# Hi-PACE/hipace

Hardware: AMD Instinct MI355X
Metric: transverse slices/s at 1024^2 x 4ppc (explicit solver) (higher is better)
Workload: dtype f64

## Files before the change

hipace_amd/csrc/multigrid.hip:

```cpp
#include "common.h"
#include <type_traits>
#include "mg_gate.h"
#include "slab_ops.h"

#include <vector>
#include <algorithm>
#include <cmath>
#include <cstring>

namespace hps {

struct FView {
    double* p; long js, ns; int oi, oj;
    __device__ __forceinline__ double& operator() (int i, int j, int n) const {
        const unsigned o = (unsigned)((i + oi) + (j + oj)*(int)js + n*(int)ns)*8u;
        return *reinterpret_cast<double*>(reinterpret_cast<char*>(p) + o);
    }
};

struct LevBox { int lox, loy, hix, hiy;
                int vlx, vly, vhx, vhy; };

enum { SRC_ZERO = 0, SRC_DIRECT = 1, SRC_PROLONG = 2 };

#define HPS_KEEP(x) asm volatile("" :: "v"(x))

#ifdef HPS_STAMPS
__device__ long long* g_mg_dbg = nullptr;
#define MG_STAMP(i) do { if (g_mg_dbg && blockIdx.x == 0 && threadIdx.x == 0) g_mg_dbg[i] = __builtin_amdgcn_s_memtime(); } while (0)
#else
#define MG_STAMP(i) do { } while (0)
#endif

template <int TX_, int TY_, int NT_>
struct TileShape {
    static constexpr int TX = TX_, TY = TY_, NT = NT_;
    static constexpr int AX = TX + 2, AY = TY + 2;
    static constexpr int PR = TX/2;
    static constexpr int GPAIRS = TX*TY/2/NT;
    static_assert(TX*TY/2 % NT == 0 && NT % 64 == 0 && (PR == 16 || PR == 32), "tile shape");
};
using TileBig = TileShape<64, 32, 512>;
using TileMid = TileShape<32, 32, 256>;
using TileHuge = TileShape<64, 48, 512>;
using TileHugeNodal = TileShape<64, 32, 512>;
template <bool CC> struct HugeTileOf { using type = TileHuge; };
template <> struct HugeTileOf<false> { using type = TileHugeNodal; };
using TileSmall = TileShape<32, 16, 256>;

template <bool CC>
__device__ __forceinline__ double diag_c0 (int i, int j, const LevBox& b, double acf, double facx, double facy)
{
    double c0 = -(acf + 2.0*(facx + facy));
    if (CC && (i == b.lox || i == b.hix)) c0 -= 2.0*facx;
    if (CC && (j == b.loy || j == b.hiy)) c0 -= 2.0*facy;
    return c0;
}

template <bool CC, bool INTERIOR = false, class P>
__device__ __forceinline__ double offdiag (P c, int sy, int i, int j, const LevBox& b, double facx, double facy)
{
    const double w = c[-1], e = c[1], s = c[-sy], n = c[sy];
    double lx = facx*(w + e), ly = facy*(s + n);
    if (CC && !INTERIOR) {
        const double fx43 = facx*(4./3.), fy43 = facy*(4./3.);
        lx = (i == b.lox) ? fx43*e : ((i == b.hix) ? fx43*w : lx);
        ly = (j == b.loy) ? fy43*n : ((j == b.hiy) ? fy43*s : ly);
    }
    return lx + ly;
}
// ... 32 lines not shown
    }
    lap += tx;
    lap += ty;
    return rhs + acf*p0 - lap;
}

template <bool CC>
__device__ __forceinline__ double prolong_at (const FView& crse, int i, int j, int n)
{
    const int ic = i >> 1, jc = j >> 1;
    if (CC) return crse(ic, jc, n);
    const bool io = (i & 1), jo = (j & 1);
    if (io && jo)  return (crse(ic, jc, n) + crse(ic+1, jc, n) + crse(ic, jc+1, n) + crse(ic+1, jc+1, n))*0.25;
    if (io)        return (crse(ic, jc, n) + crse(ic+1, jc, n))*0.5;
    if (jo)        return (crse(ic, jc, n) + crse(ic, jc+1, n))*0.5;
    return crse(ic, jc, n);
}

constexpr int MG_MAX_VCYCLES = 1024;
template <int NT>
__device__ __forceinline__ void block_max_to (unsigned long long* slot, double v, double* s_red)
{
    for (int o = 32; o > 0; o >>= 1) v = fmax(v, __shfl_xor(v, o));
    if ((threadIdx.x & 63) == 0) s_red[threadIdx.x >> 6] = v;
    __syncthreads();
    if (threadIdx.x == 0) {
        double m = 0.0;
        for (int w = 0; w < NT/64; ++w) m = fmax(m, s_red[w]);
        if (m > 0.0) atomicMax(slot + (blockIdx.x & (MG_NSUB - 1)), (unsigned long long)__double_as_longlong(m));
    }
    __syncthreads();
}

#define MG_ROWPK(m) const int jj = BR ? (tid / PR)*GPAIRS + (m) : (tid + MG_NT*(m)) / PR, pk = BR ? (tid & (PR - 1)) : (tid + MG_NT*(m)) - jj*PR
template <bool CC> __device__ __forceinline__ double restrict_at (const FView& fine, int i, int j, int n);
template <class TS, bool CC, int SRC, bool DO_RES, bool FUSE_R, bool INTERIOR, int NSW, bool GATE_IN = (NSW == 4), bool RPULL = false>
__device__ __forceinline__ void smooth_tile (double (&s_phi)[2][TS::AY*TS::AX], double* s_red, double* s_crs, const LevBox& b, const FView& phi_out,
                                             const FView& phi_out2, const FView& rhs, const FView& acf, const FView& phi_in, const FView& crse,
                                             const FView& res_out, const FView& cres_out, double facx, double facy,
                                             int gi0, int gj0, unsigned long long* resnorm, unsigned long long* rhsnorm, const StopRule& sr)
{
    constexpr int E = DO_RES ? NSW : NSW - 1;
    constexpr int GT_X = TS::TX, GT_Y = TS::TY, GA_X = TS::AX, GA_Y = TS::AY, MG_NT = TS::NT, GPAIRS = TS::GPAIRS, PR = TS::PR;
    constexpr int AXH = GA_X/2, CH = GA_Y*AXH;
    constexpr bool BR = GPAIRS <= 2 || INTERIOR;
    const int tid = threadIdx.x;
    const int cpar = (gi0 + gj0) & 1;
    MG_STAMP(0);
    double r0[GPAIRS][2], r1[GPAIRS][2], ac[GPAIRS][2], ci[GPAIRS][2];
    bool in[GPAIRS][2];
    int hx[GPAIRS];
    double fxm[GPAIRS][2], fym[GPAIRS];
    double rmax = 0.0;
#pragma unroll
    for (int m = 0; m < GPAIRS; ++m) {
        MG_ROWPK(m);
        const int j = gj0 + jj;
        hx[m] = (gi0 + 2*pk + j) & 1;
        fym[m] = INTERIOR ? facy : wall_mult<CC>(j, b.loy, b.hiy, facy);
#pragma unroll
        for (int p = 0; p < 2; ++p) {
            const int i = gi0 + 2*pk + (hx[m] ^ p);
            fxm[m][p] = INTERIOR ? facx : wall_mult<CC>(i, b.lox, b.hix, facx);
            const int ic = INTERIOR ? i : min(max(i, b.vlx), b.vhx), jc = INTERIOR ? j : min(max(j, b.vly), b.vhy);
            const bool ok = INTERIOR || (ic == i && jc == j);
            in[m][p] = ok;
            double a0, a1;
            if constexpr (RPULL) { a0 = restrict_at<CC>(crse, ic, jc, 0); a1 = restrict_at<CC>(crse, ic, jc, 1); }
            else { a0 = rhs(ic, jc, 0); a1 = rhs(ic, jc, 1); }
            const double a2 = acf(ic, jc, 0);
            r0[m][p] = ok ? a0 : 0.0;
            r1[m][p] = ok ? a1 : 0.0;
            ac[m][p] = ok ? a2 : 0.0;
            ci[m][p] = 1.0/diag_c0<CC>(i, j, b, ac[m][p], facx, facy);
            if (rhsnorm) rmax = fmax(rmax, fmax(fabs(r0[m][p]), fabs(r1[m][p])));
        }
    }
    MG_STAMP(1);
    {
        constexpr int NF = (GA_X*GA_Y + MG_NT - 1)/MG_NT;
        double v0[NF], v1[NF];
        constexpr bool PLDS = !CC && SRC == SRC_PROLONG;
        constexpr int CXN = GA_X/2 + 2, CYN = GA_Y/2 + 2;
        const int cx0 = (INTERIOR ? gi0 - 1 : min(max(gi0 - 1, b.vlx), b.vhx)) >> 1, cy0 = (INTERIOR ? gj0 - 1 : min(max(gj0 - 1, b.vly), b.vhy)) >> 1;
        if constexpr (PLDS) {
            const int cxl = b.vlx >> 1, cxh = (b.vhx >> 1) + 1, cyl = b.vly >> 1, cyh = (b.vhy >> 1) + 1;
            constexpr int NC = (CXN*CYN + MG_NT - 1)/MG_NT;
            double c0[NC], c1[NC];
#pragma unroll
            for (int m = 0; m < NC; ++m) {
                const int q = min(tid + MG_NT*m, CXN*CYN - 1);
                const int ly = q / CXN, lx = q - ly*CXN;
                const int X = min(max(cx0 + lx, cxl), cxh), Y = min(max(cy0 + ly, cyl), cyh);
                c0[m] = crse(X, Y, 0); c1[m] = crse(X, Y, 1);
            }
#pragma unroll
            for (int m = 0; m < NC; ++m) {
                const int q = tid + MG_NT*m;
                if (q < CXN*CYN) { s_crs[q] = c0[m]; s_crs[CXN*CYN + q] = c1[m]; }
            }
        }
#pragma unroll
        for (int m = 0; m < NF; ++m) {
            const int s = min(tid + MG_NT*m, GA_X*GA_Y - 1);
            const int lj = s / GA_X, li = s - lj*GA_X;
            const int i = gi0 - 1 + li, j = gj0 - 1 + lj;
            v0[m] = 0.0; v1[m] = 0.0;
            if (SRC != SRC_ZERO) {
                const int ic = INTERIOR ? i : min(max(i, b.vlx), b.vhx), jc = INTERIOR ? j : min(max(j, b.vly), b.vhy);
                double a0 = phi_in(ic, jc, 0), a1 = phi_in(ic, jc, 1);
                if (SRC == SRC_PROLONG && !PLDS) { a0 += prolong_at<CC>(crse, ic, jc, 0); a1 += prolong_at<CC>(crse, ic, jc, 1); }
                const bool inside = INTERIOR || (ic == i && jc == j);
                v0[m] = inside ? a0 : 0.0; v1[m] = inside ? a1 : 0.0;
            }
        }
        if constexpr (PLDS) {
            __syncthreads();
#pragma unroll
            for (int m = 0; m < NF; ++m) {
                const int s = min(tid + MG_NT*m, GA_X*GA_Y - 1);
                const int lj = s / GA_X, li = s - lj*GA_X;
                const int i = gi0 - 1 + li, j = gj0 - 1 + lj;
                const int ic = INTERIOR ? i : min(max(i, b.vlx), b.vhx), jc = INTERIOR ? j : min(max(j, b.vly), b.vhy);
                const bool inside = INTERIOR || (ic == i && jc == j);
                const int o = ((jc >> 1) - cy0)*CXN + (ic >> 1) - cx0;
                const bool io = (ic & 1), jo = (jc & 1);
                double p0, p1;
                const double* q0 = s_crs + o; const double* q1 = s_crs + CXN*CYN + o;
                if (io && jo)  { p0 = (q0[0] + q0[1] + q0[CXN] + q0[CXN + 1])*0.25; p1 = (q1[0] + q1[1] + q1[CXN] + q1[CXN + 1])*0.25; }
                else if (io)   { p0 = (q0[0] + q0[1])*0.5; p1 = (q1[0] + q1[1])*0.5; }
                else if (jo)   { p0 = (q0[0] + q0[CXN])*0.5; p1 = (q1[0] + q1[CXN])*0.5; }
                else           { p0 = q0[0]; p1 = q1[0]; }
                if (inside) { v0[m] += p0; v1[m] += p1; }
            }
        }
        {
            if (GATE_IN) {
                const bool active = vcycle_active(sr);
#pragma unroll
                for (int m = 0; m < GPAIRS; ++m) { HPS_KEEP(r0[m][0]); HPS_KEEP(r0[m][1]); HPS_KEEP(r1[m][0]); HPS_KEEP(r1[m][1]); HPS_KEEP(ac[m][0]); HPS_KEEP(ac[m][1]); }
#pragma unroll
                for (int m = 0; m < NF; ++m) { HPS_KEEP(v0[m]); HPS_KEEP(v1[m]); }
                if (!active) return;
            }
        }
#pragma unroll
        for (int m = 0; m < NF; ++m) {
            const int s = tid + MG_NT*m;
            if (s < GA_X*GA_Y) {
                const int lj = s / GA_X, li = s - lj*GA_X;
                const int o = ((cpar + li + lj) & 1)*CH + lj*AXH + (li >> 1);
                s_phi[0][o] = v0[m]; s_phi[1][o] = v1[m];
            }
        }
    }
    __syncthreads();
    MG_STAMP(2);

    double l0[GPAIRS][2], l1[GPAIRS][2];
    if constexpr (BR) {
#pragma unroll
        for (int m = 0; m < GPAIRS; ++m) {
            MG_ROWPK(m);
            const int row = (jj + 1)*AXH + pk;
#pragma unroll
            for (int p = 0; p < 2; ++p) { const int h = hx[m] ^ p; l0[m][p] = s_phi[0][p*CH + row + h]; l1[m][p] = s_phi[1][p*CH + row + h]; }
        }
#pragma unroll
        for (int icolor = 0; icolor < NSW; ++icolor) {
            const int p = icolor & 1;
#pragma unroll
            for (int m = 0; m < GPAIRS; ++m) {
                MG_ROWPK(m);
                const int h = hx[m] ^ p;
                const int row = (jj + 1)*AXH + pk;
                const double* nb0 = &s_phi[0][(1 - p)*CH + row];
                const double* nb1 = &s_phi[1][(1 - p)*CH + row];
                const double we0 = nb0[h] + l0[m][1 - p], we1 = nb1[h] + l1[m][1 - p];
                const double s0 = (m > 0) ? l0[m > 0 ? m - 1 : 0][1 - p] : nb0[h - AXH], s1 = (m > 0) ? l1[m > 0 ? m - 1 : 0][1 - p] : nb1[h - AXH];
                const double t0 = (m + 1 < GPAIRS) ? l0[m + 1 < GPAIRS ? m + 1 : m][1 - p] : nb0[h + AXH], t1 = (m + 1 < GPAIRS) ? l1[m + 1 < GPAIRS ? m + 1 : m][1 - p] : nb1[h + AXH];
                const double n0 = (r0[m][p] - (fxm[m][p]*we0 + fym[m]*(s0 + t0)))*ci[m][p];
                const double n1 = (r1[m][p] - (fxm[m][p]*we1 + fym[m]*(s1 + t1)))*ci[m][p];
                if (INTERIOR || in[m][p]) { s_phi[0][p*CH + row + h] = n0; s_phi[1][p*CH + row + h] = n1; l0[m][p] = n0; l1[m][p] = n1; }
            }
            __syncthreads();
        }
    } else {
#pragma unroll
        for (int icolor = 0; icolor < NSW; ++icolor) {
            constexpr int dummy = 0; (void)dummy;
            const int p = icolor & 1;
#pragma unroll
            for (int m = 0; m < GPAIRS; ++m) {
                MG_ROWPK(m);
                const int h = hx[m] ^ p;
                const int row = (jj + 1)*AXH + pk;
                const double* nb0 = &s_phi[0][(1 - p)*CH + row];
                const double* nb1 = &s_phi[1][(1 - p)*CH + row];
                const double n0 = (r0[m][p] - (fxm[m][p]*(nb0[0] + nb0[1]) + fym[m]*(nb0[h - AXH] + nb0[h + AXH])))*ci[m][p];
                const double n1 = (r1[m][p] - (fxm[m][p]*(nb1[0] + nb1[1]) + fym[m]*(nb1[h - AXH] + nb1[h + AXH])))*ci[m][p];
                if (INTERIOR || in[m][p]) { s_phi[0][p*CH + row + h] = n0; s_phi[1][p*CH + row + h] = n1; }
            }
            __syncthreads();
        }
    }
    MG_STAMP(3);

    double resmax = 0.0;
    if constexpr (BR) {
        double la0[GPAIRS], ra0[GPAIRS], la1[GPAIRS], ra1[GPAIRS];
        bool finr[GPAIRS];
#pragma unroll
        for (int m = 0; m < GPAIRS; ++m) {
            MG_ROWPK(m);
            const int j = gj0 + jj;
            const bool rowok = (jj >= E && jj < GT_Y - E);
            double q0[2], q1[2];
            bool fin[2];
#pragma unroll
            for (int p = 0; p < 2; ++p) {
                const int h = hx[m] ^ p;
                const int ii = 2*pk + h;
                fin[p] = rowok && ii >= E && ii < GT_X - E && in[m][p];
                const int i = gi0 + ii;
                const int row = (jj + 1)*AXH + pk;
                const double f0 = l0[m][p], f1 = l1[m][p];
                q0[p] = 0.0; q1[p] = 0.0;
                if (DO_RES) {
                    const double* nb0 = &s_phi[0][(1 - p)*CH + row];
                    const double* nb1 = &s_phi[1][(1 - p)*CH + row];
                    const double o0 = nb0[h], o1 = nb1[h];
                    const double w0 = h ? l0[m][1 - p] : o0, e0 = h ? o0 : l0[m][1 - p];
                    const double w1 = h ? l1[m][1 - p] : o1, e1 = h ? o1 : l1[m][1 - p];
                    const double s0 = (m > 0) ? l0[m > 0 ? m - 1 : 0][1 - p] : nb0[h - AXH], s1 = (m > 0) ? l1[m > 0 ? m - 1 : 0][1 - p] : nb1[h - AXH];
                    const double n0 = (m + 1 < GPAIRS) ? l0[m + 1 < GPAIRS ? m + 1 : m][1 - p] : nb0[h + AXH], n1 = (m + 1 < GPAIRS) ? l1[m + 1 < GPAIRS ? m + 1 : m][1 - p] : nb1[h + AXH];
                    const double t0 = residual_v<INTERIOR>(f0, w0, e0, s0, n0, i, j, b, r0[m][p], ac[m][p], facx, facy);
                    const double t1 = residual_v<INTERIOR>(f1, w1, e1, s1, n1, i, j, b, r1[m][p], ac[m][p], facx, facy);
                    q0[p] = fin[p] ? t0 : 0.0; q1[p] = fin[p] ? t1 : 0.0;
                    resmax = fmax(resmax, fmax(fabs(q0[p]), fabs(q1[p])));
                }
                if (fin[p]) {
                    if constexpr (RPULL) { rhs(i, j, 0) = r0[m][p]; rhs(i, j, 1) = r1[m][p]; }
                    if (DO_RES && !FUSE_R) { res_out(i, j, 0) = q0[p]; res_out(i, j, 1) = q1[p]; }
                    phi_out(i, j, 0) = f0;
                    phi_out(i, j, 1) = f1;
                    if (phi_out2.p) { phi_out2(i, j, 0) = f0; phi_out2(i, j, 1) = f1; }
                }
            }
            const bool sw = (hx[m] != 0);
            la0[m] = sw ? q0[1] : q0[0]; ra0[m] = sw ? q0[0] : q0[1];
            la1[m] = sw ? q1[1] : q1[0]; ra1[m] = sw ? q1[0] : q1[1];
            finr[m] = fin[0];
        }
        if (FUSE_R) {
            const double c0 = __shfl_down(la0[0], PR), d0 = __shfl_down(ra0[0], PR);
            const double c1 = __shfl_down(la1[0], PR), d1 = __shfl_down(ra1[0], PR);
#pragma unroll
            for (int m = 0; m < GPAIRS; ++m) {
                MG_ROWPK(m);
                if (finr[m] && ((jj & 1) == 0)) {
                    const bool own = (m + 1 < GPAIRS);
                    const int mu = own ? m + 1 : m;
                    const double ua0 = own ? la0[mu] : c0, ub0 = own ? ra0[mu] : d0, ua1 = own ? la1[mu] : c1, ub1 = own ? ra1[mu] : d1;
                    const int ic = (gi0 + 2*pk) >> 1, jc = (gj0 + jj) >> 1;
                    cres_out(ic, jc, 0) = 0.25*(la0[m] + ra0[m] + ua0 + ub0);
                    cres_out(ic, jc, 1) = 0.25*(la1[m] + ra1[m] + ua1 + ub1);
                }
            }
        }
    } else {
#pragma unroll
        for (int m = 0; m < GPAIRS; ++m) {
            MG_ROWPK(m);
            const int j = gj0 + jj;
            const bool rowok = (jj >= E && jj < GT_Y - E);
            double q0[2], q1[2];
            bool fin[2];
#pragma unroll
            for (int p = 0; p < 2; ++p) {
                const int h = hx[m] ^ p;
                const int ii = 2*pk + h;
                fin[p] = rowok && ii >= E && ii < GT_X - E && in[m][p];
                const int i = gi0 + ii;
                const int row = (jj + 1)*AXH + pk;
                const double f0 = s_phi[0][p*CH + row + h], f1 = s_phi[1][p*CH + row + h];
                q0[p] = 0.0; q1[p] = 0.0;
                if (DO_RES) {
                    const double* nb0 = &s_phi[0][(1 - p)*CH + row];
                    const double* nb1 = &s_phi[1][(1 - p)*CH + row];
                    const double t0 = residual_v<INTERIOR>(f0, nb0[0], nb0[1], nb0[h - AXH], nb0[h + AXH], i, j, b, r0[m][p], ac[m][p], facx, facy);
                    const double t1 = residual_v<INTERIOR>(f1, nb1[0], nb1[1], nb1[h - AXH], nb1[h + AXH], i, j, b, r1[m][p], ac[m][p], facx, facy);
                    q0[p] = fin[p] ? t0 : 0.0; q1[p] = fin[p] ? t1 : 0.0;
                    resmax = fmax(resmax, fmax(fabs(q0[p]), fabs(q1[p])));
                }
                if (fin[p]) {
                    if constexpr (RPULL) { rhs(i, j, 0) = r0[m][p]; rhs(i, j, 1) = r1[m][p]; }
                    if (DO_RES && !FUSE_R) { res_out(i, j, 0) = q0[p]; res_out(i, j, 1) = q1[p]; }
                    phi_out(i, j, 0) = f0;
                    phi_out(i, j, 1) = f1;
                    if (phi_out2.p) { phi_out2(i, j, 0) = f0; phi_out2(i, j, 1) = f1; }
                }
            }
            if (FUSE_R) {
                const bool sw = (hx[m] != 0);
                const double la0 = sw ? q0[1] : q0[0], ra0 = sw ? q0[0] : q0[1];
                const double la1 = sw ? q1[1] : q1[0], ra1 = sw ? q1[0] : q1[1];
                const double c0 = __shfl_down(la0, PR), d0 = __shfl_down(ra0, PR);
                const double c1 = __shfl_down(la1, PR), d1 = __shfl_down(ra1, PR);
                if (fin[0] && ((tid & PR) == 0)) {
                    const int ic = (gi0 + 2*pk) >> 1, jc = j >> 1;
                    cres_out(ic, jc, 0) = 0.25*(la0 + ra0 + c0 + d0);
                    cres_out(ic, jc, 1) = 0.25*(la1 + ra1 + c1 + d1);
                }
            }
        }
    }
    MG_STAMP(4);
    if (DO_RES && resnorm) block_max_to<MG_NT>(resnorm, resmax, s_red);
    if (rhsnorm) block_max_to<MG_NT>(rhsnorm, rmax, s_red);
    MG_STAMP(5);
}

template <class TS, bool CC, int SRC, bool DO_RES, bool FUSE_R, int NSW = 4, bool RPULL = false>
__global__ __launch_bounds__(TS::NT, (RPULL && TS::GPAIRS > 1) ? 2 : 4)
void k_smooth (LevBox b, FView phi_out, FView phi_out2, FView rhs, FView acf, FView phi_in, FView crse, FView res_out,
               FView cres_out, double facx, double facy, int ntx, unsigned long long* resnorm,
               unsigned long long* rhsnorm, StopRule sr)
{
    static_assert(!FUSE_R || (CC && DO_RES), "fused restriction is cell-centred only");
    if (NSW != 4 && !vcycle_active(sr)) return;
    constexpr int GT_X = TS::TX, GT_Y = TS::TY;
    __shared__ double s_phi[2][TS::AY*TS::AX];
    __shared__ double s_red[TS::NT/64];
    constexpr bool PLDS = !CC && SRC == SRC_PROLONG;
    __shared__ double s_crs[PLDS ? 2*(TS::AX/2 + 2)*(TS::AY/2 + 2) : 1];
    constexpr int E = DO_RES ? NSW : NSW - 1;
    constexpr int FX = GT_X - 2*E, FY = GT_Y - 2*E;
    const int nb = gridDim.x, q8 = nb >> 3, r8 = nb & 7, xcd = blockIdx.x & 7;
    const int tile = xcd*q8 + min(xcd, r8) + (blockIdx.x >> 3);
    const int bx = tile % ntx, by = tile / ntx;
    const int gi0 = b.vlx + bx*FX - E;
    const int gj0 = b.vly + by*FY - E;
    const bool interior = (gi0 - 1 >= b.vlx) && (gi0 + GT_X <= b.vhx) && (gj0 - 1 >= b.vly) && (gj0 + GT_Y <= b.vhy)
                       && (gi0 > b.lox) && (gi0 + GT_X - 1 < b.hix) && (gj0 > b.loy) && (gj0 + GT_Y - 1 < b.hiy);
    constexpr bool GATE_IN = (NSW == 4);
    if (interior) smooth_tile<TS, CC, SRC, DO_RES, FUSE_R, true, NSW, GATE_IN, RPULL>(s_phi, s_red, s_crs, b, phi_out, phi_out2, rhs, acf, phi_in, crse, res_out, cres_out,
                                                             facx, facy, gi0, gj0, resnorm, rhsnorm, sr);
    else          smooth_tile<TS, CC, SRC, DO_RES, FUSE_R, false, NSW, GATE_IN, RPULL>(s_phi, s_red, s_crs, b, phi_out, phi_out2, rhs, acf, phi_in, crse, res_out, cres_out,
                                                              facx, facy, gi0, gj0, resnorm, rhsnorm, sr);
}

template <bool CC>
__device__ __forceinline__ double restrict_at (const FView& fine, int i, int j, int n)
{
    if (CC) return 0.25*(fine(2*i, 2*j, n) + fine(2*i+1, 2*j, n) + fine(2*i, 2*j+1, n) + fine(2*i+1, 2*j+1, n));
    return (1./16.)*(fine(2*i-1, 2*j-1, n) + 2.*fine(2*i, 2*j-1, n) + fine(2*i+1, 2*j-1, n)
                   + 2.*fine(2*i-1, 2*j, n) + 4.*fine(2*i, 2*j, n) + 2.*fine(2*i+1, 2*j, n)
                   + fine(2*i-1, 2*j+1, n) + 2.*fine(2*i, 2*j+1, n) + fine(2*i+1, 2*j+1, n));
}

template <bool CC>
__global__ __launch_bounds__(256)
void k_restrict (LevBox cb, FView crse, FView fine, int ncomp, StopRule sr)
{
    if (!vcycle_active(sr)) return;
    const int i = cb.vlx + blockIdx.x*blockDim.x + threadIdx.x;
    const int j = cb.vly + blockIdx.y;
    if (i > cb.vhx || j > cb.vhy) return;
    for (int n = 0; n < ncomp; ++n) crse(i, j, n) = restrict_at<CC>(fine, i, j, n);
}

typedef __attribute__((address_space(3))) double lds_double;

struct LowLev { LevBox b; int nxb; int cells; int off; };

struct LView {
    lds_double* p; int nxb; int lox, loy;
    __device__ __forceinline__ lds_double& operator() (int i, int j) const { return p[(i - lox) + (j - loy)*nxb]; }
};
__device__ __forceinline__ LView lplane (lds_double* base, const LowLev& l, int plane)
{
    return LView{base + l.off + plane*l.cells, l.nxb, l.b.lox, l.b.loy};
}

template <bool CC>
__device__ __forceinline__ double lrestrict (const LView& f, int i, int j)
{
    if (CC) return 0.25*(f(2*i, 2*j) + f(2*i+1, 2*j) + f(2*i, 2*j+1) + f(2*i+1, 2*j+1));
    return (1./16.)*(f(2*i-1, 2*j-1) + 2.*f(2*i, 2*j-1) + f(2*i+1, 2*j-1)
                   + 2.*f(2*i-1, 2*j) + 4.*f(2*i, 2*j) + 2.*f(2*i+1, 2*j)
                   + f(2*i-1, 2*j+1) + 2.*f(2*i, 2*j+1) + f(2*i+1, 2*j+1));
}

template <bool CC>
__device__ __forceinline__ double lprolong (const LView& c, int i, int j)
{
    const int ic = i >> 1, jc = j >> 1;
    if (CC) return c(ic, jc);
    const bool io = (i & 1), jo = (j & 1);
    if (io && jo)  return (c(ic, jc) + c(ic+1, jc) + c(ic, jc+1) + c(ic+1, jc+1))*0.25;
    if (io)        return (c(ic, jc) + c(ic+1, jc))*0.5;
    if (jo)        return (c(ic, jc) + c(ic, jc+1))*0.5;
// ... 857 lines not shown
            e.total = off3;
            HPS_HIP_CHECK(hipMalloc(&M->coef_img, (size_t)e.ctot*sizeof(double)));
            HPS_HIP_CHECK(hipMemset(M->coef_img, 0, (size_t)e.ctot*sizeof(double)));
            M->low3_lds = (size_t)off3*sizeof(double);
            if (M->low3_lds > 64*1024)
                HPS_HIP_CHECK(hipFuncSetAttribute((const void*)k_lower_v3, hipFuncAttributeMaxDynamicSharedMemorySize, (int)M->low3_lds));
            HPS_HIP_CHECK(hipMalloc(&M->d_low3, sizeof(Low2)));
            HPS_HIP_CHECK(hipMemcpy(M->d_low3, &e, sizeof(Low2), hipMemcpyHostToDevice));
            HPS_HIP_CHECK(hipMalloc(&M->cinvA, (size_t)e.nx[0]*e.ny[0]*sizeof(double)));
            break;
        }
    }
    if (!M->use_low3) {
        long cells = 0;
        for (int il = M->lowv_begin; il < nl; ++il) cells += M->L[il].cells;
        M->low_lds = (size_t)(8*cells)*sizeof(double);
        hipFuncAttributes fa{};
        HPS_HIP_CHECK(hipFuncGetAttributes(&fa, M->cc ? (const void*)k_lower_v<true> : (const void*)k_lower_v<false>));
        if (M->low_lds + fa.sharedSizeBytes > device_max_lds()) { M->bottom = true; M->lowv_begin = nl - 1; M->low_lds = 0; }
    }
    M->nodal_pull1 = !M->cc && M->lowv_begin > 1;
    if (!M->use_low3 && !M->bottom) {
        std::vector<LowLev> low;
        int off = 0;
        for (int il = M->lowv_begin; il < nl; ++il) {
            const MGLevelDev& l = M->L[il];
            low.push_back(LowLev{l.b, l.b.hix - l.b.lox + 1, (int)l.cells, off});
            off += 8*(int)l.cells;
        }
        if (M->low_lds > 64*1024) {
            HPS_HIP_CHECK(hipFuncSetAttribute((const void*)k_lower_v<true>, hipFuncAttributeMaxDynamicSharedMemorySize, (int)M->low_lds));
            HPS_HIP_CHECK(hipFuncSetAttribute((const void*)k_lower_v<false>, hipFuncAttributeMaxDynamicSharedMemorySize, (int)M->low_lds));
        }
        HPS_HIP_CHECK(hipMalloc(&M->d_low, low.size()*sizeof(LowLev)));
        HPS_HIP_CHECK(hipMemcpy(M->d_low, low.data(), low.size()*sizeof(LowLev), hipMemcpyHostToDevice));
    }
    HPS_HIP_CHECK(hipMalloc(&M->d_buf, (3 + MG_MAX_VCYCLES)*MG_NSUB*sizeof(unsigned long long)));
    HPS_HIP_CHECK(hipHostMalloc(&M->h_buf, ((3 + MG_MAX_VCYCLES)*MG_NSUB + 8)*sizeof(unsigned long long), hipHostMallocMapped));
    HPS_HIP_CHECK(hipHostGetDevicePointer((void**)&M->h_buf_dev, M->h_buf, 0));
    M->h_seq = M->h_buf + (3 + MG_MAX_VCYCLES)*MG_NSUB; M->h_seq_dev = M->h_buf_dev + (3 + MG_MAX_VCYCLES)*MG_NSUB;
    *M->h_seq = 0ULL;
    HPS_HIP_CHECK(hipMemset(M->d_buf, 0, (3 + MG_MAX_VCYCLES)*MG_NSUB*sizeof(unsigned long long)));
    memset(M->h_buf, 0, (3 + MG_MAX_VCYCLES)*MG_NSUB*sizeof(unsigned long long));
    M->d_norms = M->d_buf + MG_NSUB; M->h_norms = M->h_buf + MG_NSUB;
    HPS_HIP_CHECK(hipMalloc(&M->tmp0, 2*M->L[0].cells*sizeof(double)));
    HPS_HIP_CHECK(hipMemset(M->tmp0, 0, 2*M->L[0].cells*sizeof(double)));
    *out = M;
    return HPS_OK;
}

template <class TS, bool CC, int SRC, bool DO_RES, int NSW = 4, bool RPULL = false>
static void launch_smooth_ts (Multigrid* M, int il, FView phi_out, FView phi_out2, FView rhs, FView acf, FView phi_in, FView crse,
                              FView res_out, FView cres_out, unsigned long long* resnorm, unsigned long long* rhsnorm,
                              const StopRule& sr, hipStream_t st)
{
    const LevBox& b = M->L[il].b;
    constexpr int E = DO_RES ? NSW : NSW - 1;
    constexpr int FX = TS::TX - 2*E, FY = TS::TY - 2*E;
    const int ntx = ceil_div(b.vhx - b.vlx + 1, FX), nty = ceil_div(b.vhy - b.vly + 1, FY);
    const double fac = (double)(1 << il);
    const double ldx = M->dx*fac, ldy = M->dy*fac;
    const double facx = 1.0/(ldx*ldx), facy = 1.0/(ldy*ldy);
    constexpr bool FUSE = CC && DO_RES;
    hipLaunchKernelGGL((k_smooth<TS, CC, SRC, DO_RES, FUSE, NSW, RPULL>), dim3(ntx*nty), dim3(TS::NT), 0, st, b, phi_out, phi_out2, rhs, acf,
                       phi_in, crse, res_out, cres_out, facx, facy, ntx, resnorm, rhsnorm, sr);
}

template <bool CC, int SRC, bool DO_RES>
static void launch_smooth (Multigrid* M, int il, FView phi_out, FView phi_out2, FView rhs, FView acf, FView phi_in, FView crse,
                           FView res_out, FView cres_out, unsigned long long* resnorm, unsigned long long* rhsnorm,
                           const StopRule& sr, hipStream_t st)
{
    if (M->L[il].cells <= SMALL_TILE_CELLS)
        launch_smooth_ts<TileSmall, CC, SRC, DO_RES>(M, il, phi_out, phi_out2, rhs, acf, phi_in, crse, res_out, cres_out, resnorm, rhsnorm, sr, st);
    else
        launch_smooth_ts<TileBig, CC, SRC, DO_RES>(M, il, phi_out, phi_out2, rhs, acf, phi_in, crse, res_out, cres_out, resnorm, rhsnorm, sr, st);
}

template <bool CC>
static void restrict_residual_if_nodal (Multigrid* M, int il, const StopRule& sr, hipStream_t st)
{
    if (CC) return;
    const LevBox& cb = M->L[il+1].b;
    hipLaunchKernelGGL(k_restrict<CC>, dim3(ceil_div(cb.vhx - cb.vlx + 1, 64), cb.vhy - cb.vly + 1), dim3(64), 0, st,
                       cb, M->lv(il+1, M->L[il+1].res), M->lv(il, M->L[il].rescor), 2, sr);
}

template <bool CC>
static void vcycle (Multigrid* M, int k, double tol_rel, double tol_abs, hipStream_t st)
{
    const int nl = M->nlev();
    const int lb = M->lowv_begin;
    const FView none{};
    const StopRule sr{M->d_norms, k, tol_rel, tol_abs};
    for (int il = 1; il < lb; ++il) {
        if (!M->pulls(il))
            launch_smooth<CC, SRC_ZERO, true>(M, il, M->lv(il, M->L[il].cor), none, M->lv(il, M->L[il].res), M->lv(il, M->L[il].acf), none,
                                              none, M->lv(il, M->L[il].rescor), M->lv(il+1, M->L[il+1].res), nullptr, nullptr, sr, st);
        else if constexpr (!CC) {
            if (M->L[il].cells > SMALL_TILE_CELLS)
                launch_smooth_ts<TileMid, CC, SRC_ZERO, true, 4, true>(M, il, M->lv(il, M->L[il].cor), none, M->lv(il, M->L[il].res), M->lv(il, M->L[il].acf), none,
                                                                       M->lv(il-1, M->L[il-1].rescor), M->lv(il, M->L[il].rescor), M->lv(il+1, M->L[il+1].res), nullptr, nullptr, sr, st);
            else
                launch_smooth_ts<TileSmall, CC, SRC_ZERO, true, 4, true>(M, il, M->lv(il, M->L[il].cor), none, M->lv(il, M->L[il].res), M->lv(il, M->L[il].acf), none,
                                                                         M->lv(il-1, M->L[il-1].rescor), M->lv(il, M->L[il].rescor), M->lv(il+1, M->L[il+1].res), nullptr, nullptr, sr, st);
        }
        if (!M->pulls(il + 1)) restrict_residual_if_nodal<CC>(M, il, sr, st);
    }
    {
        const double fac = (double)(1 << lb);
        const double ldx = M->dx*fac, ldy = M->dy*fac;
        const LevBox& bb = M->L[nl-1].b;
        const int nsweeps = std::max(16, (std::max(bb.hix - bb.lox + 1, bb.hiy - bb.loy + 1) + 1)/2*2);
        if (M->bottom) {
            const FView cor = M->lv(lb, M->L[lb].cor), rhs = M->lv(lb, M->L[lb].res), acf = M->lv(lb, M->L[lb].acf);
            const dim3 grid(ceil_div(bb.vhx - bb.vlx + 1, 64), bb.vhy - bb.vly + 1);
            for (int is = -1; is < nsweeps; ++is)
                hipLaunchKernelGGL(k_bottom_sweep<CC>, grid, dim3(64), 0, st, bb, cor, rhs, acf, 1.0/(ldx*ldx), 1.0/(ldy*ldy), is, sr);
        } else if (M->use_low3)
            hipLaunchKernelGGL(k_lower_v3, dim3(2), dim3(1024), M->low3_lds, st, M->d_low3, M->L[lb].acf, M->cinvA, M->L[lb].res, M->L[lb].cor,
                               M->coef_img, M->low3.nx[0], M->low3.ny[0], M->low3.ctot, 1.0/(ldx*ldx), 1.0/(ldy*ldy), nsweeps, sr);
        else
            hipLaunchKernelGGL(k_lower_v<CC>, dim3(CC ? 1 : 2), dim3(1024), M->low_lds, st, M->d_low, nl - lb, M->L[lb].acf, M->L[lb].res,
                               M->L[lb].cor, 1.0/(ldx*ldx), 1.0/(ldy*ldy), nsweeps, sr, M->pulls(lb) ? M->lv(lb-1, M->L[lb-1].rescor) : FView{});
    }
    for (int il = lb - 1; il >= 1; --il) {
        double* crse = (il + 1 == lb) ? M->L[il+1].cor : M->L[il+1].rescor;
        launch_smooth<CC, SRC_PROLONG, false>(M, il, M->lv(il, M->L[il].rescor), none, M->lv(il, M->L[il].res), M->lv(il, M->L[il].acf),
                                              M->lv(il, M->L[il].cor), M->lv(il+1, crse), none, none, nullptr, nullptr, sr, st);
    }
    {
        double* crse = (1 == lb) ? M->L[1].cor : M->L[1].rescor;
        double* in = M->cor_in_tmp ? M->tmp0 : M->L[0].cor;
        double* out = M->cor_in_tmp ? M->L[0].cor : M->tmp0;
        launch_smooth_ts<typename HugeTileOf<CC>::type, CC, SRC_PROLONG, true, 8>(M, 0, M->lv(0, out), M->sol, M->rhs, M->acf0, M->lv(0, in), M->lv(1, crse),
                                                             M->lv(0, M->L[0].rescor), M->lv(1, M->L[1].res), M->d_norms + (2 + k)*MG_NSUB,
                                                             nullptr, sr, st);
        M->cor_in_tmp = !M->cor_in_tmp;
    }
    if (!M->nodal_pull1) restrict_residual_if_nodal<CC>(M, 0, sr, st);
}

__global__ __launch_bounds__(256)
void k_post_norms (const unsigned long long* __restrict__ src, volatile unsigned long long* dst, int nwords,
                   volatile unsigned long long* seq_slot, unsigned long long seq, int* go_word, StopRule after)
{
    {   const bool act = vcycle_active(after);
        if (threadIdx.x == 0) *go_word = act ? 0 : 1; }
    for (int w = threadIdx.x; w < nwords; w += blockDim.x) dst[w] = src[w];
    HPS_HOST_STORES_ACKNOWLEDGED();
    __syncthreads();
    if (threadIdx.x == 0) { *seq_slot = seq; }
}

template <bool CC>
static void enqueue_cycles (Multigrid* M, hipStream_t st)
{
    SolveRun& r = M->run;
    for (int v = 0; v < r.nspec && r.enq < r.max_iters; ++v, ++r.enq) {
        if (r.enq >= r.nzeroed) {
            const int more = std::min(r.max_iters - r.nzeroed, 64);
            (void)hipMemsetAsync(M->d_norms + (2 + r.nzeroed)*MG_NSUB, 0, more*MG_NSUB*sizeof(unsigned long long), st);
            r.nzeroed += more;
        }
        vcycle<CC>(M, r.enq, r.tol_rel, r.tol_abs, st);
    }
    ++M->seq; ++M->dbg_trips;
    if (M->defer_post) {
        M->defer_post = false; M->deferred_valid = true;
        M->deferred = MgPost{M->d_buf, (volatile unsigned long long*)M->h_buf_dev, (3 + r.enq)*MG_NSUB, (volatile unsigned long long*)M->h_seq_dev, M->seq,
                             StopRule{M->d_norms, r.enq, r.tol_rel, r.tol_abs}};
        return;
    }
    hipLaunchKernelGGL(k_post_norms, dim3(1), dim3(256), 0, st, M->d_buf, (volatile unsigned long long*)M->h_buf_dev,
                       (3 + r.enq)*MG_NSUB, (volatile unsigned long long*)M->h_seq_dev, M->seq,
                       reinterpret_cast<int*>(M->d_buf) + MG_GO_WORD, StopRule{M->d_norms, r.enq, r.tol_rel, r.tol_abs});
}

struct GuestPass { bool on = false; SlabView f{hps_slab{}}; GradPsiSxSy ga{}; };

template <bool CC>
static int solve1_hierarchy (Multigrid* M, int max_iters, hipStream_t st, const GuestPass* guest = nullptr)
{
    const int lb = M->lowv_begin;
    max_iters = std::min(max_iters, MG_MAX_VCYCLES);
    const StopRule always{nullptr, -1, 0.0, 0.0};
    int nspec = std::min(std::max(M->last_iters, 1), std::max(max_iters, 1));
    int nzeroed = std::min(max_iters, nspec + 8);
    const int nzero_words = (2 + nzeroed)*MG_NSUB;
    int first = 1;
    if (CC) {
        PyrOut po{};
        const int np = std::min(lb, 5);
        for (int il = 1; il <= np; ++il) { po.p[il-1] = M->L[il].acf; po.nx[il-1] = M->L[il].b.hix + 1; po.ny[il-1] = M->L[il].b.hiy + 1; }
        const double lfac = (double)(1 << lb), lfx = 1.0/(M->dx*lfac*M->dx*lfac), lfy = 1.0/(M->dy*lfac*M->dy*lfac);
        if (M->use_low3 && lb <= np) { po.cinv = M->cinvA; po.cinv_l = lb - 1; po.cfx = lfx; po.cfy = lfy; }
        if (guest) {
            const int gx = ceil_div(M->nx, 32), gy = ceil_div(M->ny, 32);
            const SlabView& f = guest->f;
            const int nbx = ceil_div(f.js, 256), rows = f.ny + 2*f.ng;
            hipLaunchKernelGGL(k_hierarchy_gradpsi, dim3(gx*gy + nbx*rows), dim3(256), 0, st, M->acf0, M->nx, M->ny, po, np, M->d_norms, nzero_words,
                               gx, gy, f, guest->ga, nbx);
        } else
        hipLaunchKernelGGL(k_acf_pyramid, dim3(ceil_div(M->nx, 32), ceil_div(M->ny, 32)), dim3(256), 0, st, M->acf0, M->nx, M->ny, po, np,
                           M->d_norms, nzero_words);
        first = np + 1;
    } else {
        NodalPyr o{};
        const int np = std::min(lb, NPYR_MAX);
        o.np = np;
        o.vhx[0] = M->L[0].b.vhx; o.vhy[0] = M->L[0].b.vhy;
        for (int il = 1; il <= np; ++il) { o.lev[il-1] = M->lv(il, M->L[il].acf); o.vhx[il] = M->L[il].b.vhx; o.vhy[il] = M->L[il].b.vhy; }
        const int tx = ceil_div(M->L[np].b.hix, NPYR_NB), ty = ceil_div(M->L[np].b.hiy, NPYR_NB);
        switch (np) {
            case 1: hipLaunchKernelGGL(k_nodal_acf_pyramid<1>, dim3(tx, ty), dim3(256), nodal_pyramid_lds(np), st, M->acf0, o, M->d_norms, nzero_words); break;
            case 2: hipLaunchKernelGGL(k_nodal_acf_pyramid<2>, dim3(tx, ty), dim3(256), nodal_pyramid_lds(np), st, M->acf0, o, M->d_norms, nzero_words); break;
            case 3: hipLaunchKernelGGL(k_nodal_acf_pyramid<3>, dim3(tx, ty), dim3(256), nodal_pyramid_lds(np), st, M->acf0, o, M->d_norms, nzero_words); break;
            case 4: hipLaunchKernelGGL(k_nodal_acf_pyramid<4>, dim3(tx, ty), dim3(256), nodal_pyramid_lds(np), st, M->acf0, o, M->d_norms, nzero_words); break;
// ... 274 lines not shown
```

Baseline: 1678.

## Specialize interior smoother addressing, defer slab writes to last V-cycle of batch

Interior tiles now compute global addresses from precomputed byte offsets plus row strides, and the halo fill uses a wave-aligned row mapping instead of per-element div/mod. The inverse-diagonal and rhs-norm work moves behind the activity gate. Tile index decode now uses a reciprocal multiply, and the interior test uses host-precomputed tile ranges. The fine-level write of the solution slab (phi_out2) is skipped except on the last V-cycle in a speculative batch, with a fallback copy kernel path when a cycle turns out inactive. This adds complexity and a risk that the solution slab is stale when the batch stops early.

```diff
diff --git a/hipace_amd/csrc/multigrid.hip b/hipace_amd/csrc/multigrid.hip
--- a/hipace_amd/csrc/multigrid.hip
+++ b/hipace_amd/csrc/multigrid.hip
@@ -16,6 +16,10 @@
         const unsigned o = (unsigned)((i + oi) + (j + oj)*(int)js + n*(int)ns)*8u;
         return *reinterpret_cast<double*>(reinterpret_cast<char*>(p) + o);
     }
+    __device__ __forceinline__ unsigned off (int i, int j) const { return (unsigned)((i + oi) + (j + oj)*(int)js)*8u; }
+    __device__ __forceinline__ unsigned rowb () const { return (unsigned)(int)js*8u; }
+    __device__ __forceinline__ unsigned compb () const { return (unsigned)(int)ns*8u; }
+    __device__ __forceinline__ double& at (unsigned o) const { return *reinterpret_cast<double*>(reinterpret_cast<char*>(p) + o); }
 };
 
 struct LevBox { int lox, loy, hix, hiy;
@@ -154,18 +158,53 @@
     int hx[GPAIRS];
     double fxm[GPAIRS][2], fym[GPAIRS];
     double rmax = 0.0;
+    const int bpk = tid & (PR - 1), bj0 = (tid / PR)*GPAIRS;
+    const int hx0 = (gi0 + gj0 + bj0) & 1;
+    const unsigned h8 = (unsigned)hx0*8u;
+#define MG_PAIRSEL(m, p, base) (((((m) & 1) ^ (p)) ? (base) + 8u - h8 : (base) + h8))
 #pragma unroll
     for (int m = 0; m < GPAIRS; ++m) {
+        if constexpr (INTERIOR) {
+            static_assert(BR, "interior tiles sweep in block rows");
+            hx[m] = hx0 ^ (m & 1);
+            fym[m] = facy;
+            const unsigned rb = RPULL ? crse.off(2*(gi0 + 2*bpk), 2*(gj0 + bj0)) : rhs.off(gi0 + 2*bpk, gj0 + bj0);
+            const unsigned ab = acf.off(gi0 + 2*bpk, gj0 + bj0);
+#pragma unroll
+            for (int p = 0; p < 2; ++p) {
+                fxm[m][p] = facx;
+                in[m][p] = true;
+                if constexpr (RPULL) {
+                    const unsigned rw = crse.rowb(), o = (((m & 1) ^ p) ? rb + 16u - 2u*h8 : rb + 2u*h8) + (unsigned)(2*m)*rw;
+#pragma unroll
+                    for (int n = 0; n < 2; ++n) {
+                        const unsigned c = o + (unsigned)n*crse.compb();
+                        const double v = (1./16.)*(crse.at(c - rw - 8u) + 2.*crse.at(c - rw) + crse.at(c - rw + 8u)
+                                                 + 2.*crse.at(c - 8u) + 4.*crse.at(c) + 2.*crse.at(c + 8u)
+                                                 + crse.at(c + rw - 8u) + 2.*crse.at(c + rw) + crse.at(c + rw + 8u));
+                        if (n == 0) r0[m][p] = v; else r1[m][p] = v;
+                    }
+                } else {
+                    const unsigned o = MG_PAIRSEL(m, p, rb) + (unsigned)m*rhs.rowb();
+                    r0[m][p] = rhs.at(o); r1[m][p] = rhs.at(o + rhs.compb());
+                }
+                ac[m][p] = acf.at(MG_PAIRSEL(m, p, ab) + (unsigned)m*acf.rowb());
+                if constexpr (!GATE_IN) {
+                    ci[m][p] = 1.0/diag_c0<false>(0, 0, b, ac[m][p], facx, facy);
+                    if (rhsnorm) rmax = fmax(rmax, fmax(fabs(r0[m][p]), fabs(r1[m][p])));
+                }
+            }
+        } else {
         MG_ROWPK(m);
         const int j = gj0 + jj;
         hx[m] = (gi0 + 2*pk + j) & 1;
-        fym[m] = INTERIOR ? facy : wall_mult<CC>(j, b.loy, b.hiy, facy);
+        fym[m] = wall_mult<CC>(j, b.loy, b.hiy, facy);
 #pragma unroll
         for (int p = 0; p < 2; ++p) {
             const int i = gi0 + 2*pk + (hx[m] ^ p);
-            fxm[m][p] = INTERIOR ? facx : wall_mult<CC>(i, b.lox, b.hix, facx);
-            const int ic = INTERIOR ? i : min(max(i, b.vlx), b.vhx), jc = INTERIOR ? j : min(max(j, b.vly), b.vhy);
-            const bool ok = INTERIOR || (ic == i && jc == j);
+            fxm[m][p] = wall_mult<CC>(i, b.lox, b.hix, facx);
+            const int ic = min(max(i, b.vlx), b.vhx), jc = min(max(j, b.vly), b.vhy);
+            const bool ok = (ic == i && jc == j);
             in[m][p] = ok;
             double a0, a1;
             if constexpr (RPULL) { a0 = restrict_at<CC>(crse, ic, jc, 0); a1 = restrict_at<CC>(crse, ic, jc, 1); }
@@ -174,14 +213,25 @@
             r0[m][p] = ok ? a0 : 0.0;
             r1[m][p] = ok ? a1 : 0.0;
             ac[m][p] = ok ? a2 : 0.0;
-            ci[m][p] = 1.0/diag_c0<CC>(i, j, b, ac[m][p], facx, facy);
-            if (rhsnorm) rmax = fmax(rmax, fmax(fabs(r0[m][p]), fabs(r1[m][p])));
+            if constexpr (!GATE_IN) {
+                ci[m][p] = 1.0/diag_c0<CC>(i, j, b, ac[m][p], facx, facy);
+                if (rhsnorm) rmax = fmax(rmax, fmax(fabs(r0[m][p]), fabs(r1[m][p])));
+            }
+        }
         }
     }
     MG_STAMP(1);
     {
         constexpr int NF = (GA_X*GA_Y + MG_NT - 1)/MG_NT;
         double v0[NF], v1[NF];
+        constexpr int NW = MG_NT/64, RPW = 64/GT_X, RSTEP = NW*RPW, NFR = GA_Y/RSTEP, RW = (GA_Y - NFR*RSTEP)/RPW;
+        static_assert(NF == NFR + 1 && GA_Y - NFR*RSTEP == 2 && RSTEP % 2 == 0 && RW + 2 <= NW && GA_Y <= 64 && GA_X == GT_X + 2, "fill mapping");
+        const int wv = __builtin_amdgcn_readfirstlane(tid >> 6), ln = tid & 63;
+        const int fcol = ln & (GT_X - 1), frow = wv*RPW + ln/GT_X;
+        const bool strip = wv >= RW;
+        const int li_l = strip ? GT_X + ((wv - RW) & 1) : fcol, lj_l = strip ? min(ln, GA_Y - 1) : frow + NFR*RSTEP;
+        const bool val_l = !strip || (wv < RW + 2 && ln < GA_Y);
+#define MG_FILL_CELL(m) const int li = (m) < NFR ? fcol : li_l, lj = (m) < NFR ? frow + (m)*RSTEP : lj_l
         constexpr bool PLDS = !CC && SRC == SRC_PROLONG;
         constexpr int CXN = GA_X/2 + 2, CYN = GA_Y/2 + 2;
         const int cx0 = (INTERIOR ? gi0 - 1 : min(max(gi0 - 1, b.vlx), b.vhx)) >> 1, cy0 = (INTERIOR ? gj0 - 1 : min(max(gj0 - 1, b.vly), b.vhy)) >> 1;
@@ -204,24 +254,33 @@
         }
 #pragma unroll
         for (int m = 0; m < NF; ++m) {
-            const int s = min(tid + MG_NT*m, GA_X*GA_Y - 1);
-            const int lj = s / GA_X, li = s - lj*GA_X;
+            MG_FILL_CELL(m);
             const int i = gi0 - 1 + li, j = gj0 - 1 + lj;
             v0[m] = 0.0; v1[m] = 0.0;
             if (SRC != SRC_ZERO) {
-                const int ic = INTERIOR ? i : min(max(i, b.vlx), b.vhx), jc = INTERIOR ? j : min(max(j, b.vly), b.vhy);
+                if constexpr (INTERIOR) {
+                    const unsigned o = (m < NFR) ? phi_in.off(gi0 - 1 + fcol, gj0 - 1 + frow) + (unsigned)(m*RSTEP)*phi_in.rowb() : phi_in.off(i, j);
+                    double a0 = phi_in.at(o), a1 = phi_in.at(o + phi_in.compb());
+                    if (SRC == SRC_PROLONG && !PLDS) {
+                        const unsigned c = (m < NFR) ? crse.off((gi0 - 1 + fcol) >> 1, (gj0 - 1 + frow) >> 1) + (unsigned)(m*(RSTEP/2))*crse.rowb()
+                                                     : crse.off(i >> 1, j >> 1);
+                        a0 += crse.at(c); a1 += crse.at(c + crse.compb());
+                    }
+                    v0[m] = a0; v1[m] = a1;
+                } else {
+                const int ic = min(max(i, b.vlx), b.vhx), jc = min(max(j, b.vly), b.vhy);
                 double a0 = phi_in(ic, jc, 0), a1 = phi_in(ic, jc, 1);
                 if (SRC == SRC_PROLONG && !PLDS) { a0 += prolong_at<CC>(crse, ic, jc, 0); a1 += prolong_at<CC>(crse, ic, jc, 1); }
-                const bool inside = INTERIOR || (ic == i && jc == j);
+                const bool inside = (ic == i && jc == j);
                 v0[m] = inside ? a0 : 0.0; v1[m] = inside ? a1 : 0.0;
+                }
             }
         }
         if constexpr (PLDS) {
             __syncthreads();
 #pragma unroll
             for (int m = 0; m < NF; ++m) {
-                const int s = min(tid + MG_NT*m, GA_X*GA_Y - 1);
-                const int lj = s / GA_X, li = s - lj*GA_X;
+                MG_FILL_CELL(m);
                 const int i = gi0 - 1 + li, j = gj0 - 1 + lj;
                 const int ic = INTERIOR ? i : min(max(i, b.vlx), b.vhx), jc = INTERIOR ? j : min(max(j, b.vly), b.vhy);
                 const bool inside = INTERIOR || (ic == i && jc == j);
@@ -243,18 +302,29 @@
                 for (int m = 0; m < GPAIRS; ++m) { HPS_KEEP(r0[m][0]); HPS_KEEP(r0[m][1]); HPS_KEEP(r1[m][0]); HPS_KEEP(r1[m][1]); HPS_KEEP(ac[m][0]); HPS_KEEP(ac[m][1]); }
 #pragma unroll
                 for (int m = 0; m < NF; ++m) { HPS_KEEP(v0[m]); HPS_KEEP(v1[m]); }
-                if (!active) return;
-            }
-        }
-#pragma unroll
-        for (int m = 0; m < NF; ++m) {
-            const int s = tid + MG_NT*m;
-            if (s < GA_X*GA_Y) {
-                const int lj = s / GA_X, li = s - lj*GA_X;
-                const int o = ((cpar + li + lj) & 1)*CH + lj*AXH + (li >> 1);
-                s_phi[0][o] = v0[m]; s_phi[1][o] = v1[m];
-            }
-        }
+                if (__builtin_expect(!active, 0)) return;
+#pragma unroll
+                for (int m = 0; m < GPAIRS; ++m) {
+                    MG_ROWPK(m);
+#pragma unroll
+                    for (int p = 0; p < 2; ++p)
+                        ci[m][p] = INTERIOR ? 1.0/diag_c0<false>(0, 0, b, ac[m][p], facx, facy)
+                                            : 1.0/diag_c0<CC>(gi0 + 2*pk + (hx[m] ^ p), gj0 + jj, b, ac[m][p], facx, facy);
+                }
+                if (rhsnorm) {
+#pragma unroll
+                    for (int m = 0; m < GPAIRS; ++m) { rmax = fmax(rmax, fmax(fabs(r0[m][0]), fabs(r1[m][0]))); rmax = fmax(rmax, fmax(fabs(r0[m][1]), fabs(r1[m][1]))); }
+                }
+            }
+        }
+        const int so = ((cpar + fcol + frow) & 1)*CH + frow*AXH + (fcol >> 1);
+#pragma unroll
+        for (int m = 0; m < NFR; ++m) { s_phi[0][so + m*RSTEP*AXH] = v0[m]; s_phi[1][so + m*RSTEP*AXH] = v1[m]; }
+        if (val_l) {
+            const int o = ((cpar + li_l + lj_l) & 1)*CH + lj_l*AXH + (li_l >> 1);
+            s_phi[0][o] = v0[NFR]; s_phi[1][o] = v1[NFR];
+        }
+#undef MG_FILL_CELL
     }
     __syncthreads();
     MG_STAMP(2);
@@ -342,11 +412,12 @@
                     resmax = fmax(resmax, fmax(fabs(q0[p]), fabs(q1[p])));
                 }
                 if (fin[p]) {
-                    if constexpr (RPULL) { rhs(i, j, 0) = r0[m][p]; rhs(i, j, 1) = r1[m][p]; }
-                    if (DO_RES && !FUSE_R) { res_out(i, j, 0) = q0[p]; res_out(i, j, 1) = q1[p]; }
-                    phi_out(i, j, 0) = f0;
-                    phi_out(i, j, 1) = f1;
-                    if (phi_out2.p) { phi_out2(i, j, 0) = f0; phi_out2(i, j, 1) = f1; }
+                    if constexpr (RPULL) { const unsigned o = MG_PAIRSEL(m, p, rhs.off(gi0 + 2*bpk, gj0 + bj0)) + (unsigned)m*rhs.rowb(); rhs.at(o) = r0[m][p]; rhs.at(o + rhs.compb()) = r1[m][p]; }
+                    if (DO_RES && !FUSE_R) { const unsigned o = MG_PAIRSEL(m, p, res_out.off(gi0 + 2*bpk, gj0 + bj0)) + (unsigned)m*res_out.rowb(); res_out.at(o) = q0[p]; res_out.at(o + res_out.compb()) = q1[p]; }
+                    const unsigned o = MG_PAIRSEL(m, p, phi_out.off(gi0 + 2*bpk, gj0 + bj0)) + (unsigned)m*phi_out.rowb();
+                    phi_out.at(o) = f0;
+                    phi_out.at(o + phi_out.compb()) = f1;
+                    if (phi_out2.p) { const unsigned o2 = MG_PAIRSEL(m, p, phi_out2.off(gi0 + 2*bpk, gj0 + bj0)) + (unsigned)m*phi_out2.rowb(); phi_out2.at(o2) = f0; phi_out2.at(o2 + phi_out2.compb()) = f1; }
                 }
             }
             const bool sw = (hx[m] != 0);
@@ -359,14 +430,14 @@
             const double c1 = __shfl_down(la1[0], PR), d1 = __shfl_down(ra1[0], PR);
 #pragma unroll
             for (int m = 0; m < GPAIRS; ++m) {
-                MG_ROWPK(m);
+                const int jj = bj0 + m;
                 if (finr[m] && ((jj & 1) == 0)) {
                     const bool own = (m + 1 < GPAIRS);
                     const int mu = own ? m + 1 : m;
                     const double ua0 = own ? la0[mu] : c0, ub0 = own ? ra0[mu] : d0, ua1 = own ? la1[mu] : c1, ub1 = own ? ra1[mu] : d1;
-                    const int ic = (gi0 + 2*pk) >> 1, jc = (gj0 + jj) >> 1;
-                    cres_out(ic, jc, 0) = 0.25*(la0[m] + ra0[m] + ua0 + ub0);
-                    cres_out(ic, jc, 1) = 0.25*(la1[m] + ra1[m] + ua1 + ub1);
+                    const unsigned o = cres_out.off((gi0 >> 1) + bpk, (gj0 + bj0) >> 1) + (unsigned)((m + 1) >> 1)*cres_out.rowb();
+                    cres_out.at(o) = 0.25*(la0[m] + ra0[m] + ua0 + ub0);
+                    cres_out.at(o + cres_out.compb()) = 0.25*(la1[m] + ra1[m] + ua1 + ub1);
                 }
             }
         }
@@ -417,39 +488,55 @@
             }
         }
     }
+#undef MG_PAIRSEL
+    (void)bpk; (void)bj0; (void)h8;
     MG_STAMP(4);
     if (DO_RES && resnorm) block_max_to<MG_NT>(resnorm, resmax, s_red);
     if (rhsnorm) block_max_to<MG_NT>(rhsnorm, rmax, s_red);
     MG_STAMP(5);
 }
 
+struct TileMap { int ntx; unsigned rcp; int q8; short r8, slab; short ix0, ix1, iy0, iy1; };
+enum { MG_SLAB_WRITE = 1 };
+
 template <class TS, bool CC, int SRC, bool DO_RES, bool FUSE_R, int NSW = 4, bool RPULL = false>
 __global__ __launch_bounds__(TS::NT, (RPULL && TS::GPAIRS > 1) ? 2 : 4)
 void k_smooth (LevBox b, FView phi_out, FView phi_out2, FView rhs, FView acf, FView phi_in, FView crse, FView res_out,
-               FView cres_out, double facx, double facy, int ntx, unsigned long long* resnorm,
+               FView cres_out, double facx, double facy, TileMap tm, unsigned long long* resnorm,
                unsigned long long* rhsnorm, StopRule sr)
 {
     static_assert(!FUSE_R || (CC && DO_RES), "fused restriction is cell-centred only");
-    if (NSW != 4 && !vcycle_active(sr)) return;
     constexpr int GT_X = TS::TX, GT_Y = TS::TY;
-    __shared__ double s_phi[2][TS::AY*TS::AX];
-    __shared__ double s_red[TS::NT/64];
-    constexpr bool PLDS = !CC && SRC == SRC_PROLONG;
-    __shared__ double s_crs[PLDS ? 2*(TS::AX/2 + 2)*(TS::AY/2 + 2) : 1];
     constexpr int E = DO_RES ? NSW : NSW - 1;
     constexpr int FX = GT_X - 2*E, FY = GT_Y - 2*E;
-    const int nb = gridDim.x, q8 = nb >> 3, r8 = nb & 7, xcd = blockIdx.x & 7;
-    const int tile = xcd*q8 + min(xcd, r8) + (blockIdx.x >> 3);
-    const int bx = tile % ntx, by = tile / ntx;
-    const int gi0 = b.vlx + bx*FX - E;
-    const int gj0 = b.vly + by*FY - E;
-    const bool interior = (gi0 - 1 >= b.vlx) && (gi0 + GT_X <= b.vhx) && (gj0 - 1 >= b.vly) && (gj0 + GT_Y <= b.vhy)
-                       && (gi0 > b.lox) && (gi0 + GT_X - 1 < b.hix) && (gj0 > b.loy) && (gj0 + GT_Y - 1 < b.hiy);
-    constexpr bool GATE_IN = (NSW == 4);
-    if (interior) smooth_tile<TS, CC, SRC, DO_RES, FUSE_R, true, NSW, GATE_IN, RPULL>(s_phi, s_red, s_crs, b, phi_out, phi_out2, rhs, acf, phi_in, crse, res_out, cres_out,
-                                                             facx, facy, gi0, gj0, resnorm, rhsnorm, sr);
-    else          smooth_tile<TS, CC, SRC, DO_RES, FUSE_R, false, NSW, GATE_IN, RPULL>(s_phi, s_red, s_crs, b, phi_out, phi_out2, rhs, acf, phi_in, crse, res_out, cres_out,
-                                                              facx, facy, gi0, gj0, resnorm, rhsnorm, sr);
+    const int xcd = blockIdx.x & 7;
+    const int tile = xcd*tm.q8 + min(xcd, tm.r8) + (blockIdx.x >> 3);
+    int by = (int)__umulhi((unsigned)tile, tm.rcp);
+    if ((unsigned)(tile - by*tm.ntx) >= (unsigned)tm.ntx) ++by;
+    const int bx = tile - by*tm.ntx;
+    if (__builtin_expect(NSW == 4 || vcycle_active(sr), 1)) {
+        if (!(tm.slab & MG_SLAB_WRITE)) phi_out2.p = nullptr;
+        __shared__ double s_phi[2][TS::AY*TS::AX];
+        __shared__ double s_red[TS::NT/64];
+        constexpr bool PLDS = !CC && SRC == SRC_PROLONG;
+        __shared__ double s_crs[PLDS ? 2*(TS::AX/2 + 2)*(TS::AY/2 + 2) : 1];
+        const int gi0 = b.vlx + bx*FX - E;
+        const int gj0 = b.vly + by*FY - E;
+        const bool interior = bx >= tm.ix0 && bx <= tm.ix1 && by >= tm.iy0 && by <= tm.iy1;
+        constexpr bool GATE_IN = (NSW == 4);
+        if (interior) smooth_tile<TS, CC, SRC, DO_RES, FUSE_R, true, NSW, GATE_IN, RPULL>(s_phi, s_red, s_crs, b, phi_out, phi_out2, rhs, acf, phi_in, crse, res_out, cres_out,
+                                                                 facx, facy, gi0, gj0, resnorm, rhsnorm, sr);
+        else          smooth_tile<TS, CC, SRC, DO_RES, FUSE_R, false, NSW, GATE_IN, RPULL>(s_phi, s_red, s_crs, b, phi_out, phi_out2, rhs, acf, phi_in, crse, res_out, cres_out,
+                                                                  facx, facy, gi0, gj0, resnorm, rhsnorm, sr);
+        return;
+    }
+    if (NSW == 8 && sr.k >= 1 && phi_out2.p && vcycle_active(StopRule{sr.norms, sr.k - 1, sr.tol_rel, sr.tol_abs})) {
+        const int i0 = b.vlx + bx*FX, j0 = b.vly + by*FY;
+        for (int t = threadIdx.x; t < FX*FY; t += TS::NT) {
+            const int i = i0 + t % FX, j = j0 + t / FX;
+            if (i <= b.vhx && j <= b.vhy) { phi_out2(i, j, 0) = phi_in(i, j, 0); phi_out2(i, j, 1) = phi_in(i, j, 1); }
+        }
+    }
 }
 
 template <bool CC>
@@ -1413,7 +1500,7 @@
 template <class TS, bool CC, int SRC, bool DO_RES, int NSW = 4, bool RPULL = false>
 static void launch_smooth_ts (Multigrid* M, int il, FView phi_out, FView phi_out2, FView rhs, FView acf, FView phi_in, FView crse,
                               FView res_out, FView cres_out, unsigned long long* resnorm, unsigned long long* rhsnorm,
-                              const StopRule& sr, hipStream_t st)
+                              const StopRule& sr, hipStream_t st, int slab = MG_SLAB_WRITE)
 {
     const LevBox& b = M->L[il].b;
     constexpr int E = DO_RES ? NSW : NSW - 1;
@@ -1423,8 +1510,21 @@
     const double ldx = M->dx*fac, ldy = M->dy*fac;
     const double facx = 1.0/(ldx*ldx), facy = 1.0/(ldy*ldy);
     constexpr bool FUSE = CC && DO_RES;
+    auto inner = [] (int n, int vl, int vh, int lo, int hi, int F, int T, short& first, short& last) {
+        first = 1; last = 0;
+        n = std::min(n, 32767);
+        for (int t = 0; t < n; ++t) {
+            const int g0 = vl + t*F - E;
+            if (g0 - 1 >= vl && g0 + T <= vh && g0 > lo && g0 + T - 1 < hi) { if (first > last) first = (short)t; last = (short)t; }
+        }
+    };
+    TileMap tm{};
+    tm.ntx = ntx; tm.rcp = (unsigned)std::min<unsigned long long>((1ULL << 32)/(unsigned)ntx, 0xffffffffULL);
+    tm.q8 = (ntx*nty) >> 3; tm.r8 = (short)((ntx*nty) & 7); tm.slab = (short)slab;
+    inner(ntx, b.vlx, b.vhx, b.lox, b.hix, FX, TS::TX, tm.ix0, tm.ix1);
+    inner(nty, b.vly, b.vhy, b.loy, b.hiy, FY, TS::TY, tm.iy0, tm.iy1);
     hipLaunchKernelGGL((k_smooth<TS, CC, SRC, DO_RES, FUSE, NSW, RPULL>), dim3(ntx*nty), dim3(TS::NT), 0, st, b, phi_out, phi_out2, rhs, acf,
-                       phi_in, crse, res_out, cres_out, facx, facy, ntx, resnorm, rhsnorm, sr);
+                       phi_in, crse, res_out, cres_out, facx, facy, tm, resnorm, rhsnorm, sr);
 }
 
 template <bool CC, int SRC, bool DO_RES>
@@ -1448,7 +1548,7 @@
 }
 
 template <bool CC>
-static void vcycle (Multigrid* M, int k, double tol_rel, double tol_abs, hipStream_t st)
+static void vcycle (Multigrid* M, int k, double tol_rel, double tol_abs, hipStream_t st, bool last_of_batch)
 {
     const int nl = M->nlev();
     const int lb = M->lowv_begin;
@@ -1496,7 +1596,7 @@
         double* out = M->cor_in_tmp ? M->L[0].cor : M->tmp0;
         launch_smooth_ts<typename HugeTileOf<CC>::type, CC, SRC_PROLONG, true, 8>(M, 0, M->lv(0, out), M->sol, M->rhs, M->acf0, M->lv(0, in), M->lv(1, crse),
                                                              M->lv(0, M->L[0].rescor), M->lv(1, M->L[1].res), M->d_norms + (2 + k)*MG_NSUB,
-                                                             nullptr, sr, st);
+                                                             nullptr, sr, st, last_of_batch ? MG_SLAB_WRITE : 0);
         M->cor_in_tmp = !M->cor_in_tmp;
     }
     if (!M->nodal_pull1) restrict_residual_if_nodal<CC>(M, 0, sr, st);
@@ -1524,7 +1624,7 @@
             (void)hipMemsetAsync(M->d_norms + (2 + r.nzeroed)*MG_NSUB, 0, more*MG_NSUB*sizeof(unsigned long long), st);
             r.nzeroed += more;
         }
-        vcycle<CC>(M, r.enq, r.tol_rel, r.tol_abs, st);
+        vcycle<CC>(M, r.enq, r.tol_rel, r.tol_abs, st, v + 1 == r.nspec || r.enq + 1 >= r.max_iters);
     }
     ++M->seq; ++M->dbg_trips;
     if (M->defer_post) {
```

New measurement: 1689, median of 6. No clear change (+0.7%).
